# Arief-AK/OpenCL-Development-Real-time-Image-Processing

Hardware: AMD Instinct MI355X
Metric: Mpixels/s (Gaussian 5x5, 4K RGBA) (higher is better)
Workload: dtype u8 in/out, f32 accumulate

## Files before the change

opencl-development-real-time-image-processing_amd/csrc/gauss_exact.hip:

```cpp
#include <type_traits>

#include "common.hpp"
#include "exact_common.hpp"
#include "kernels.hpp"
#include "slide_common.hpp"

namespace mi355 {

namespace {

template <int R, bool CLAMP>
__global__ __launch_bounds__(kSlideWavesPerBlock * 64) void gauss_exact_kernel(
    const uint8_t* __restrict__ in, uint8_t* __restrict__ out, int w, int h, int nstrips, int lanes_out, BandPlan plan,
    ExactTables<2 * R + 1> tab, uint32_t alpha255)
{
    constexpr int K = 2 * R + 1;
    __shared__ float flat[256];
    flat[threadIdx.x] = flat_chain<K>((float)threadIdx.x, tab.w2);
    __syncthreads();
    const int lane = threadIdx.x & 63;
    SlideItem it;
    if (!slide_item(plan, nstrips, h, &it))
        return;
    const bool up = (it.band & 1) != 0;
    const SlideGeom G = slide_geom<4>(it.strip, lanes_out, lane, w, 16u, 16u);
    const BandWalk W = band_walk(up, it.y0, it.nout, R, h);
    const int nin = W.nin, nout = it.nout;

    const size_t row_bytes = (size_t)w * 4;
    const auto fin = uniform_ptr(in + it.frame * row_bytes * h);
    const auto fout = uniform_ptr(out + it.frame * row_bytes * h);
    uint32_t in_off = G.in_off, out_off = G.out_off;

    float wv[R + 1];
#pragma unroll
    for (int d = 0; d <= R; d++)
        wv[d] = tab.w1[R - d];
// ... 85 lines not shown
    constexpr int K = 2 * R + 1;
    const StripPlan sp = make_strip_plan(w);
    BandPlan plan;
    constexpr int kRows = (R == 1) ? 16 : (R == 2 ? 24 : 40);
    constexpr int kWavesPerSimd = (R == 1) ? 5 : (R == 2 ? 3 : 2);
    if (!make_band_plan(h, sp.nstrips, nframes, kWavesPerSimd, kRows, kRows, kRows, 0.0, kRows / 2, &plan))
        return hipErrorInvalidValue;
    double wsum;
    const ExactTables<K> tab = make_exact_tables<K>(coef, &wsum);
    float chain = 0.0f;
    for (int j = 0; j < K * K; j++)
        chain += 255.0f * coef.h_w2d[j];
    chain = chain < 0.0f ? 0.0f : (chain > 255.0f ? 255.0f : chain);
    const uint32_t alpha255 = (uint32_t)chain << 24;
    return dispatch_bool(gauss_upper_clamp(wsum, 0.01), [&](auto CL) {
        return launch_slide(gauss_exact_kernel<R, CL.value>, plan, stream, d_in, d_out, w, h, sp.nstrips, sp.lanes_out,
                            plan, tab, alpha255);
    });
}

}

bool gauss_exact_supported(const uint8_t* d_in, const uint8_t* d_out, int w, int h, const GaussCoef& coef)
{
    (void)h;
    const int k = coef.k;
    if (k != 3 && k != 5 && k != 7)
        return false;
    if (rows_ragged(w, d_in, 16, d_out, 16))
        return false;
    return exact_tables_ok(coef);
}
// ... 10 lines not shown
```

opencl-development-real-time-image-processing_amd/csrc/gauss_slide.hip:

```cpp
#include <cmath>
#include <cstdlib>
#include <type_traits>

#include "common.hpp"
#include "kernels.hpp"
#include "slide_common.hpp"

namespace mi355 {

namespace {

constexpr uint32_t kRowStoreNowhere = 0x80000000u;
__device__ __forceinline__ void gstore_row_nt(global_ptr<uint8_t> rowp, uint32_t row_bytes, uint32_t off, u32x4 v)
{
    const auto rsrc = __builtin_amdgcn_make_buffer_rsrc((void*)rowp, (short)0, (int)row_bytes, 0x00020000);
    __builtin_amdgcn_raw_buffer_store_b128(v, rsrc, (int)off, 0, 2 );
}

constexpr uint32_t kSlideLdsForFiveWaves = 160u * 1024u / 5u - 1024u;
template <typename... KArgs, typename... Args>
hipError_t launch_slide_lds(void (*kernel)(KArgs...), const BandPlan& plan, uint32_t lds_bytes, hipStream_t stream,
                            Args... args)
{
    hipLaunchKernelGGL(kernel, dim3(plan.nblocks_a + plan.nblocks_b), dim3(kSlideWavesPerBlock * 64), lds_bytes, stream,
                       static_cast<KArgs>(args)...);
    return hipGetLastError();
}

template <int K>
struct Weights {
    float w[K];
};

__device__ __forceinline__ float ubyte_f32(uint32_t p, int c)
{
    return (float)((p >> (8 * c)) & 0xFFu);
}

__device__ __forceinline__ void cvt_pack4x4(const float (&h)[4][4] , u32x4& o)
{
    uint32_t o0, o1, o2, o3;
    asm("v_cvt_u32_f32_e32 %0, %4\n\t"
// ... 94 lines not shown
        : "=&v"(o0), "=&v"(o1), "=&v"(o2), "=&v"(o3)
        : "v"(v0), "v"(v1), "v"(v2), "v"(v3), "v"(w0), "v"(w1), "v"(w2), "v"(w3), "v"(w4));
}

struct SlideLane {
    global_ptr<const uint8_t> fin;
    global_ptr<uint8_t> fout;
    size_t row_bytes;
    SlideGeom g;
    int y0, nout, h;
    uint32_t px_off[4];
    int w;
    RaggedEdge edge;
};

template <bool NA0>
__device__ __forceinline__ bool alpha_row_differs(const u32x4& p, uint32_t nA)
{
    uint32_t t;
    if constexpr (NA0)
        t = (p.x & p.y) & (p.z & p.w);
    else
        t = ((p.x ^ nA) & (p.y ^ nA)) & ((p.z ^ nA) & (p.w ^ nA));
    return __builtin_amdgcn_ballot_w64(t < 0xFF000000u) != 0;
}

constexpr int kBandDone = 0;
constexpr int kBandAbortUniform = 1;
constexpr int kBandAbort = 2;
constexpr int kBandAbortUniformFirst = 3;
// ... 12 lines not shown

template <int R, bool CLAMP, int NCH, bool RAGGED, bool UP, int AMODE, bool LOCKSTEP>
__device__ __forceinline__ int gauss_slide_band(const SlideLane& L, const float (&wv)[2 * R + 1], uint32_t alpha_hi,
                                                const uint32_t* __restrict__ alpha_tab, u32x4 (&q3)[2 * R + 1],
                                                bool preloaded)
{
    constexpr int K = 2 * R + 1;
    static_assert((NCH == 4) == (AMODE == 0), "AMODE 1 / 2 belong to the 3-channel pass");
    uint32_t in_off = L.g.in_off, out_off = L.g.out_off;
    [[maybe_unused]] const uint32_t out_voff = L.g.stores ? out_off : kRowStoreNowhere;
    const BandWalk W = band_walk(UP, L.y0, L.nout, R, L.h);
    uint32_t cur_nA = 0u;
    int run = 0;
    int code = kBandDone;
    const ptrdiff_t step_bytes = UP ? -(ptrdiff_t)L.row_bytes : (ptrdiff_t)L.row_bytes;
    const int y_lo = max(L.y0 - R, 0), y_hi = min(L.y0 + L.nout - 1 + R, L.h - 1);
    int y_in = W.y_first;
    auto in_p = L.fin + (size_t)clampi(y_in, y_lo, y_hi) * L.row_bytes;
    auto out_p = L.fout + (size_t)out_row(W, 0) * L.row_bytes;
    auto next_in_row = [&]() {
        const int y_next = y_in + W.y_step;
        in_p += (min(y_in, y_next) >= y_lo && max(y_in, y_next) <= y_hi) ? step_bytes : (ptrdiff_t)0;
        y_in = y_next;
    };
    auto load_row = [&]() -> u32x4 {
        const auto rowp = in_p;
        next_in_row();
        if constexpr (R <= 2)
            lane_offset_here(in_off);
        if constexpr (RAGGED) {
            if (L.w < 4) {
                u32x4 r;
#pragma unroll
                for (int j = 0; j < 4; j++)
                    r[j] = gload<uint32_t>(rowp + L.px_off[j]);
                return r;
            }
            return gload_a4<u32x4>(rowp + in_off);
        } else {
            return gload<u32x4>(rowp + in_off);
        }
    };

    constexpr int PF = (K < 3) ? K : 3;
    u32x4 q_own[K];
    u32x4 (&q)[K] = (AMODE == 0) ? q_own : q3;
    if (AMODE != 2 || !preloaded) {
#pragma unroll
        for (int u = 0; u < PF; u++)
            q[u] = load_row();
    } else {
#pragma unroll
        for (int u = 0; u < PF; u++)
            next_in_row();
    }
    if constexpr (AMODE == 1) {
        if (alpha_row_differs<true>(q[0], 0u)) {
            const uint32_t a_row = ((uint32_t)__builtin_amdgcn_readfirstlane((int)q[0].x) >> 24) & 0xFFu;
            return alpha_row_differs<false>(q[0], (a_row ^ 0xFFu) << 24) ? kBandAbort : kBandAbortUniformFirst;
        }
    }

    constexpr bool kRing = R <= 3;
    static_assert(kRing || !UP, "the accumulator form walks down only");
    float rows[K][4 * NCH] = {};

    auto do_row = [&](auto slot, auto outputs) __attribute__((always_inline)) {
        constexpr int u = decltype(slot)::value;
        constexpr bool OUT = decltype(outputs)::value;
// ... 162 lines not shown
        constexpr int V = decltype(v)::value;
        if constexpr (V < K - 1) {
            if (V < rem) {
                do_row(std::integral_constant<int, (2 * R + V) % K>{}, std::true_type{});
                self(self, std::integral_constant<int, V + 1>{});
            }
        }
    };
    if (code == kBandDone)
        rem_rows(rem_rows, std::integral_constant<int, 0>{});
    return code;
}

template <int R, bool CLAMP, bool RAGGED, int MODE, bool LOCKSTEP>
__global__ __launch_bounds__(kSlideWavesPerBlock * 64, (R == 3 && MODE == 3) ? 3 : 1) void gauss_slide_kernel(
    const uint8_t* __restrict__ in, uint8_t* __restrict__ out, int w, int h, int nstrips, int lanes_out,
    BandPlan plan, Weights<2 * R + 1> wts, uint32_t alpha_hi, const uint32_t* __restrict__ alpha_tab,
    uint32_t* __restrict__ flags)
{
    constexpr int K = 2 * R + 1;
    const int lane = threadIdx.x & 63;
    SlideItem it;
    if (!slide_item(plan, nstrips, h, &it))
        return;
    if constexpr (MODE == 4) {
        if (flags[it.work] == 0)
            return;
    }
    SlideLane L;
    L.g = slide_geom<4>(it.strip, lanes_out, lane, w, 16u, 16u);
    L.y0 = it.y0;
    L.nout = it.nout;
    L.h = h;
    L.w = w;
    L.row_bytes = (size_t)w * 4;
    L.fin = uniform_ptr(in + it.frame * L.row_bytes * h);
    L.fout = uniform_ptr(out + it.frame * L.row_bytes * h);
    L.edge = RaggedEdge{false, false, false, false};
    if constexpr (RAGGED) {
        if (w >= 4)
            L.g.in_off = ragged_edge_setup(L.g.q_lane, L.g.q_load, w, &L.edge);
    }
#pragma unroll
    for (int j = 0; j < 4; j++)
        L.px_off[j] = (uint32_t)clampi(L.g.x_lane + j, 0, w - 1) * 4u;

    float wv[K];
#pragma unroll
    for (int j = 0; j < K; j++) {
        wv[j] = wts.w[j];
        asm volatile("" : "+v"(wv[j]));
    }

    const bool up = (it.band & 1) != 0;
    u32x4 q3[K];
    auto run = [&](auto amode, bool preloaded) -> int {
        constexpr int AMODE = decltype(amode)::value;
        constexpr int NCH = AMODE == 0 ? 4 : 3;
        if constexpr (R <= 3) {
            if (up)
                return gauss_slide_band<R, CLAMP, NCH, RAGGED, true, AMODE, LOCKSTEP>(L, wv, alpha_hi, alpha_tab, q3, preloaded);
        }
        return gauss_slide_band<R, CLAMP, NCH, RAGGED, false, AMODE, LOCKSTEP>(L, wv, alpha_hi, alpha_tab, q3, preloaded);
    };
    auto three_channels = [&]() -> int {
        int code = run(std::integral_constant<int, 1>{}, false);
        if (code == kBandAbortUniform || code == kBandAbortUniformFirst)
            code = run(std::integral_constant<int, 2>{}, code == kBandAbortUniformFirst);
        return code;
    };
    if constexpr (MODE == 0) {
        if (three_channels() != kBandDone)
            run(std::integral_constant<int, 0>{}, false);
    } else if constexpr (MODE == 3) {
        const int code = three_channels();
        if (lane == 0)
            flags[it.work] = code == kBandDone ? 0u : 1u;
    } else {
        run(std::integral_constant<int, 0>{}, false);
    }
}
// ... 26 lines not shown
    const int nstrips = sp.nstrips, lanes_out = sp.lanes_out;
    Weights<K> wts;
    for (int j = 0; j < K; j++)
        wts.w[j] = coef.h_w1d[j];
    double wsum = 0.0;
    for (int j = 0; j < K; j++)
        wsum += (double)coef.h_w1d[j];
    if (!coef.d_alpha_tab)
        return hipErrorInvalidValue;
    const uint32_t alpha_hi = coef.h_alpha_tab[255];
    const uint32_t* alpha_tab = coef.d_alpha_tab;
    const bool lockstep =
        R <= 2 && !ragged && nstrips % kSlideWavesPerBlock == 0 && plan.nwork_b == 0 && plan.nwork_a >= 8192u;
    const uint32_t lds_bytes = (R == 1 && !ragged) ? kSlideLdsForFiveWaves : 0u;
    auto launch = [&](auto kernel) {
        return launch_slide_lds(kernel, plan, lds_bytes, stream, d_in, d_out, w, h, nstrips, lanes_out, plan, wts, alpha_hi,
                                alpha_tab, d_flags);
    };
    return dispatch_bool(gauss_upper_clamp(wsum), [&](auto CL) {
        return dispatch_bool(ragged, [&](auto RG) {
            if constexpr (kSplit) {
                const hipError_t e = launch(gauss_slide_kernel<R, CL.value, RG.value, 3, false>);
                return e != hipSuccess ? e : launch(gauss_slide_kernel<R, CL.value, RG.value, 4, false>);
            } else if constexpr (RG.value) {
                return launch(gauss_slide_kernel<R, CL.value, true, 0, false>);
            } else {
                return dispatch_bool(
                    lockstep, [&](auto LS) { return launch(gauss_slide_kernel<R, CL.value, false, 0, LS.value>); });
            }
        });
    });
}
// ... 32 lines not shown
```

opencl-development-real-time-image-processing_amd/csrc/gauss_wide.hip:

```cpp
#include <cmath>

#include "common.hpp"
#include "kernels.hpp"
#include "slide_common.hpp"

namespace mi355 {

namespace {

template <int K>
struct WWeights {
    float w[K];
};

struct WideLane {
    const uint8_t* fin;
    uint8_t* fout;
    f32x4* vr;
    size_t row_bytes;
    SlideGeom g;
    int y0, nout, nin, h, lane;
};

template <int R, int NCH>
// ... 80 lines not shown
                    for (int c = 0; c < NCH; c++) {
                        r.x = __builtin_amdgcn_cvt_pk_u8_f32(__builtin_floorf(o0[c]), (uint32_t)c, r.x);
                        r.y = __builtin_amdgcn_cvt_pk_u8_f32(__builtin_floorf(o1[c]), (uint32_t)c, r.y);
                    }
                    __builtin_nontemporal_store(
                        r, reinterpret_cast<u32x2*>(L.fout + (size_t)out_row(W, m) * L.row_bytes + L.g.out_off));
                }
            }
        }
    }
    return true;
}

template <int R, int NCH>
__global__ __launch_bounds__(kSlideWavesPerBlock * 64, (NCH == 3 && R <= 6) ? 3 : 2) void gauss_wide_kernel(
    const uint8_t* __restrict__ in, uint8_t* __restrict__ out, int pairs , int h, int nstrips,
    int lanes_out, BandPlan plan, WWeights<2 * R + 1> wts, uint32_t alpha_hi, uint32_t* __restrict__ flags)
{
    constexpr int K = 2 * R + 1;
    constexpr int H = (R + 1) / 2;
    __shared__ f32x4 vrow[kSlideWavesPerBlock][128 + 2 * R + 2];
    SlideItem it;
    if (!slide_item(plan, nstrips, h, &it))
        return;
    if constexpr (NCH == 4) {
        if (flags[it.work] == 0)
            return;
    }
    WideLane L;
    L.vr = vrow[threadIdx.x >> 6];
    L.lane = threadIdx.x & 63;
    L.g = slide_geom<2, H, false>(it.strip, lanes_out, L.lane, 2 * pairs, 8u, 8u);
    L.y0 = it.y0;
    L.nout = it.nout;
    L.nin = it.nout + 2 * R;
    L.h = h;
    L.row_bytes = (size_t)pairs * 8;
    L.fin = in + it.frame * L.row_bytes * h;
// ... 26 lines not shown
hipError_t launch_r(hipStream_t stream, const uint8_t* d_in, uint8_t* d_out, int w, int h, int nframes,
                    const GaussCoef& coef, uint32_t* d_flags)
{
    constexpr int K = 2 * R + 1;
    int pairs, nstrips, lanes_out;
    BandPlan plan;
    if (!d_flags || !wide_plan<R>(w, h, nframes, pairs, nstrips, lanes_out, &plan))
        return hipErrorInvalidValue;
    WWeights<K> wts;
    for (int j = 0; j < K; j++)
        wts.w[j] = coef.h_w1d[j];
    if (!coef.d_alpha_tab)
        return hipErrorInvalidValue;
    const uint32_t alpha_hi = coef.h_alpha_tab[255];
    auto launch = [&](auto kernel) {
        return launch_slide(kernel, plan, stream, d_in, d_out, pairs, h, nstrips, lanes_out, plan, wts, alpha_hi,
                            d_flags);
    };
    const hipError_t e = launch(gauss_wide_kernel<R, 3>);
    return e != hipSuccess ? e : launch(gauss_wide_kernel<R, 4>);
}

}

bool gauss_wide_supported(const uint8_t* d_in, const uint8_t* d_out, int w, int h, int k)
{
    (void)h;
    if (k != 11 && k != 13 && k != 15 && k != 17)
        return false;
    if ((w & 1) != 0)
        return false;
    return aligned_to(d_in, 8) && aligned_to(d_out, 8);
// ... 25 lines not shown
```

opencl-development-real-time-image-processing_amd/csrc/gray.hip:

```cpp
#include <cstdlib>

#include "common.hpp"
#include "kernels.hpp"
#include "slide_common.hpp"

namespace mi355 {

namespace {

constexpr int kGrayThreads = 256;
constexpr int kGrayIlp = 4;

__device__ __forceinline__ uint32_t luma_fast_u32(uint32_t px) { return (uint32_t)luma_px_fast(px); }

__device__ __forceinline__ uint32_t pack4(uint32_t a, uint32_t b, uint32_t c, uint32_t d)
{
    return a | (b << 8) | (c << 16) | (d << 24);
}

template <bool ONE_CH>
__global__ __launch_bounds__(kGrayThreads) void gray_vec_kernel(const u32x4* __restrict__ in,
                                                                void* __restrict__ out,
                                                                size_t nquads)
{
// ... 27 lines not shown
        if constexpr (ONE_CH) {
            reinterpret_cast<uint32_t*>(out)[i] = pack4(g0, g1, g2, g3);
        } else {
            u32x4 o;
            o.x = gray_to_rgba(g0);
            o.y = gray_to_rgba(g1);
            o.z = gray_to_rgba(g2);
            o.w = gray_to_rgba(g3);
            reinterpret_cast<u32x4*>(out)[i] = o;
        }
    }
}

template <bool ONE_CH>
__global__ __launch_bounds__(kSlideWavesPerBlock * 64) void gray_strip_kernel(
    const uint8_t* __restrict__ in, uint8_t* __restrict__ out, int quads, int h, int nstrips, BandPlan plan)
{
    SlideItem it;
    if (!slide_item(plan, nstrips, h, &it))
        return;
    const int lane = threadIdx.x & 63;
    const int q = it.strip * 64 + lane;
    if (q >= quads)
        return;
    const size_t row_in = (size_t)quads * 16, row_out = ONE_CH ? (size_t)quads * 4 : row_in;
    const auto fin = uniform_ptr(in + it.frame * row_in * h);
    const auto fout = uniform_ptr(out + it.frame * row_out * h);
    uint32_t in_off = (uint32_t)q * 16u, out_off = (uint32_t)q * (ONE_CH ? 4u : 16u);
    constexpr int U = 4;
    for (int r0 = 0; r0 < it.nout; r0 += U) {
        u32x4 p[U];
#pragma unroll
        for (int u = 0; u < U; u++) {
            const int y = it.y0 + min(r0 + u, it.nout - 1);
// ... 63 lines not shown
        return (e && atoi(e) > 0) ? (unsigned)atoi(e) : (1u << 20);
    }();
    static const bool kStripForced = tune_env("MI355_TUNE_GRAY_STRIP") != nullptr;
    static const int kStripRows = [] {
        const char* e = tune_env("MI355_TUNE_GRAY_STRIP");
        return e ? atoi(e) : 4;
    }();
    const int strip_quads = w / 4, strip_n = (strip_quads + 63) / 64;
    const bool strip_ok = (w & 3) == 0 && (kStripForced || (strip_quads * 100 >= strip_n * 64 * 93 && npx >= ((size_t)1 << 28)));
    if (nquads && kStripRows > 0 && strip_ok) {
        const int quads = strip_quads, nstrips = strip_n;
        BandPlan plan;
        if (!make_band_plan(h, nstrips, nframes, 8, kStripRows, kStripRows, kStripRows, 0.0, 0, &plan))
            return hipErrorInvalidValue;
        return dispatch_bool(one_channel, [&](auto ONE_CH) {
            return launch_slide(gray_strip_kernel<ONE_CH.value>, plan, stream, d_in, d_out, quads, h, nstrips, plan);
        });
    }
    if (nquads) {
        const unsigned grid = grid_for(nquads, kGrayThreads * kGrayIlp, kCap);
        if (one_channel)
            hipLaunchKernelGGL(gray_vec_kernel<true>, dim3(grid), dim3(kGrayThreads), 0, stream,
                               reinterpret_cast<const u32x4*>(d_in), (void*)d_out, nquads);
        else
            hipLaunchKernelGGL(gray_vec_kernel<false>, dim3(grid), dim3(kGrayThreads), 0, stream,
                               reinterpret_cast<const u32x4*>(d_in), (void*)d_out, nquads);
    }
    const size_t done = nquads * 4;
    if (done < npx) {
        const unsigned grid = grid_for(npx - done, kGrayThreads, kCap);
        if (one_channel)
// ... 11 lines not shown
```

opencl-development-real-time-image-processing_amd/csrc/pipe_slide.hip:

```cpp
#include <cmath>
#include <cstdlib>

#include "common.hpp"
#include "kernels.hpp"
#include "slide_common.hpp"
#include "exact_common.hpp"

namespace mi355 {

namespace {

template <int PX>
struct PixRow {
    u32x4 v[PX / 4];
};

template <int R, int PX, bool CLAMP, bool RAGGED>
__global__ __launch_bounds__(kSlideWavesPerBlock * 64, PX == 8 ? 4 : 1) void pipe_slide_kernel(
    const uint8_t* __restrict__ in, uint8_t* __restrict__ out, int w, int h, int nstrips,
    int lanes_out, BandPlan plan, ExactTables<2 * R + 1> tab)
{
    static_assert(PX == 4 || (PX == 8 && !RAGGED), "8 pixels per lane: aligned rows only");
    constexpr int K = 2 * R + 1;
    __shared__ uint8_t lut[256];
    __shared__ float flat[256];
    lut[threadIdx.x] = (uint8_t)luma_rgb(threadIdx.x, threadIdx.x, threadIdx.x);
    flat[threadIdx.x] = flat_chain<K>((float)threadIdx.x, tab.w2);
    __syncthreads();

    const int lane = threadIdx.x & 63;
    SlideItem it;
    if (!slide_item(plan, nstrips, h, &it))
        return;
    const int y0 = it.y0, nout = it.nout;
    const bool up = (it.band & 1) != 0;

    const SlideGeom G = slide_geom<PX>(it.strip, lanes_out, lane, w, 4u * PX, (uint32_t)PX);
    const int jw = w - G.x_lane;
    const int keep_px = (lane == 0) ? PX - 1 : ((G.q_lane == G.q_end) ? 0 : -1);

    const BandWalk W = band_walk(up, y0, nout, R + 1, h);
    const int nin = W.nin;

    const size_t row_bytes = (size_t)w * 4;
    const auto fin = uniform_ptr(in + it.frame * row_bytes * h);
    const auto fout = uniform_ptr(out + it.frame * (size_t)w * h);
    uint32_t in_off = G.in_off, out_off = G.out_off;
// ... 194 lines not shown
    } else {
        const StripPlan sp = make_strip_plan(w);
        nstrips = sp.nstrips;
        lanes_out = sp.lanes_out;
        constexpr int kRows = (R == 1) ? 16 : (R == 2 ? 24 : 40);
        planned = make_band_plan(h, nstrips, nframes, 8, kRows, kRows, kRows, 0.0, kRows / 2, &plan);
    }
    if (!planned)
        return hipErrorInvalidValue;
    double wsum;
    const ExactTables<K> tab = make_exact_tables<K>(coef, &wsum);
    const bool ragged = PX == 4 && rows_ragged(w, d_in, 16, d_out, 4);
    return dispatch_bool(gauss_upper_clamp(wsum), [&](auto CL) {
        return dispatch_bool(ragged, [&](auto RG) {
            if constexpr (PX == 4 || !RG.value)
                return launch_slide(pipe_slide_kernel<R, PX, CL.value, RG.value>, plan, stream, d_in, d_out, w, h,
                                    nstrips, lanes_out, plan, tab);
            else
                return hipErrorInvalidValue;
        });
    });
}

}

bool pipe_slide_supported(const uint8_t* d_in, const uint8_t* d_out, int w, int h, const GaussCoef& coef, int px)
{
    const int k = coef.k;
    if (k != 3 && k != 5 && k != 7)
        return false;
    if (w < 4 || h < 2 || !exact_tables_ok(coef) || !aligned_to(d_in, 4))
        return false;
// ... 22 lines not shown
```

opencl-development-real-time-image-processing_amd/csrc/slide_common.hpp:

```cpp
#pragma once
#include <cstdint>
#include <cstdlib>

#include "common.hpp"

namespace mi355 {

constexpr int kSlideLanesOutMax = 62;
constexpr int kSlideWavesPerBlock = 4;

struct BandPlan {
    int rows_a, nbands_a, rows_b, nbands_b, y_split;
    uint32_t nwork_a, nwork_b, nblocks_a, nblocks_b;
};

struct StripPlan {
    int quads, nstrips, lanes_out;
};

inline StripPlan make_strip_plan(int w, int lanes_pref = 0)
{
    StripPlan s;
    s.quads = (w + 3) / 4;
    s.nstrips = (s.quads + kSlideLanesOutMax - 1) / kSlideLanesOutMax;
    s.lanes_out = (s.quads + s.nstrips - 1) / s.nstrips;
    if (lanes_pref > 0 && lanes_pref <= kSlideLanesOutMax && s.nstrips > 1) {
        s.lanes_out = lanes_pref;
        s.nstrips = (s.quads + lanes_pref - 1) / lanes_pref;
// ... 47 lines not shown
    p.y_split = h_a;
    if (h_b > 0) {
        p.nbands_b = (h_b + rows_tail - 1) / rows_tail;
        p.rows_b = (h_b + p.nbands_b - 1) / p.nbands_b;
    } else {
        p.nbands_b = 0;
        p.rows_b = 1;
    }
    const size_t na = (size_t)nstrips * p.nbands_a * nframes, nb = (size_t)nstrips * p.nbands_b * nframes;
    if (na + nb > 0x3FFFFFFFull)
        return false;
    p.nwork_a = (uint32_t)na;
    p.nwork_b = (uint32_t)nb;
    p.nblocks_a = (p.nwork_a + kSlideWavesPerBlock - 1) / kSlideWavesPerBlock;
    p.nblocks_b = (p.nwork_b + kSlideWavesPerBlock - 1) / kSlideWavesPerBlock;
    *out = p;
    return true;
}

#ifdef __HIPCC__
template <typename... KArgs, typename... Args>
hipError_t launch_slide(void (*kernel)(KArgs...), const BandPlan& plan, hipStream_t stream, Args... args)
{
    hipLaunchKernelGGL(kernel, dim3(plan.nblocks_a + plan.nblocks_b), dim3(kSlideWavesPerBlock * 64), 0, stream,
                       static_cast<KArgs>(args)...);
    return hipGetLastError();
}

template <typename T>
using global_ptr = __attribute__((address_space(1))) T*;

template <typename T>
__device__ __forceinline__ global_ptr<T> uniform_ptr(T* p)
{
    const uint64_t v = reinterpret_cast<uint64_t>(p);
    const uint32_t lo = __builtin_amdgcn_readfirstlane((uint32_t)v);
    const uint32_t hi = __builtin_amdgcn_readfirstlane((uint32_t)(v >> 32));
    return (global_ptr<T>)(((uint64_t)hi << 32) | lo);
}

__device__ __forceinline__ void lane_offset_here(uint32_t& off)
// ... 41 lines not shown
    const int shift = 4 * q_lane - xs;
    e->sh1 = shift >= 1;
    e->sh2 = shift >= 2;
    e->sh3 = shift >= 3;
    e->sh4 = shift >= 4;
    return (uint32_t)xs * 4u;
}

__device__ __forceinline__ void ragged_shift_clamp(u32x4& p, const RaggedEdge& e)
{
    p.x = e.sh3 ? p.w : (e.sh2 ? p.z : (e.sh1 ? p.y : p.x));
    p.y = e.sh2 ? p.w : (e.sh1 ? p.z : p.y);
    p.z = e.sh1 ? p.w : p.z;
}

struct SlideItem {
    int strip, band, y0, nout;
    uint32_t work;
    size_t frame;
};

__device__ __forceinline__ bool slide_item(const BandPlan& plan, int nstrips, int h, SlideItem* it)
{
    const bool tail = blockIdx.x >= plan.nblocks_a;
    const uint32_t blk = tail ? xcd_remap(blockIdx.x - plan.nblocks_a, plan.nblocks_b)
                              : xcd_remap(blockIdx.x, plan.nblocks_a);
    const uint32_t work =
        __builtin_amdgcn_readfirstlane(blk * kSlideWavesPerBlock + (uint32_t)(threadIdx.x >> 6));
    if (work >= (tail ? plan.nwork_b : plan.nwork_a))
        return false;
    const int nbands = tail ? plan.nbands_b : plan.nbands_a;
    const int band_rows = tail ? plan.rows_b : plan.rows_a;
    it->work = tail ? plan.nwork_a + work : work;
    it->strip = work % nstrips;
    const int band = (work / nstrips) % nbands;
    it->frame = work / ((uint32_t)nstrips * nbands);
    it->band = band;
    it->y0 = (tail ? plan.y_split : 0) + band * band_rows;
    it->nout = min(band_rows, (tail ? h : plan.y_split) - it->y0);
    return true;
}

struct SlideGeom {
    int q_lane, q_load, q_end, x_lane;
    bool left_of_image, right_of_image, edge_strip, stores;
    uint32_t in_off, out_off;
};

template <int PX, int HALO = 1, bool CAP_LOAD = true>
__device__ __forceinline__ SlideGeom slide_geom(int strip, int lanes_out, int lane, int w, uint32_t bytes_in,
                                                uint32_t bytes_out)
{
    static_assert(HALO == 1 || !CAP_LOAD, "the cap is written for one halo lane");
    const int quads = (w + PX - 1) >> (PX == 8 ? 3 : (PX == 4 ? 2 : 1));
    SlideGeom g;
    g.q_lane = strip * lanes_out + lane - HALO;
    g.q_load = clampi(g.q_lane, 0, CAP_LOAD ? min(quads - 1, (strip + 1) * lanes_out) : quads - 1);
    g.q_end = min((strip + 1) * lanes_out, quads);
    g.x_lane = PX * g.q_lane;
    g.left_of_image = g.q_lane < 0;
    g.right_of_image = g.q_lane >= quads;
    g.edge_strip = (strip == 0) || (PX * (strip * lanes_out + 64 - HALO) > w);
    g.stores = (lane >= HALO) && (g.q_lane < g.q_end);
    g.in_off = (uint32_t)g.q_load * bytes_in;
    g.out_off = (uint32_t)(g.stores ? g.q_lane : 0) * bytes_out;
    return g;
}

struct BandWalk {
    int y_first, y_step, halo, nin, h;
};

// ... 68 lines not shown
```

opencl-development-real-time-image-processing_amd/csrc/sobel_slide.hip:

```cpp
#include <cstdlib>

#include "common.hpp"
#include "kernels.hpp"
#include "slide_common.hpp"

namespace mi355 {

namespace {

template <bool RAGGED, bool LOCKSTEP>
__global__ __launch_bounds__(kSlideWavesPerBlock * 64) void sobel_slide_kernel(
    const uint8_t* __restrict__ in, uint8_t* __restrict__ out, int w, int h, int nstrips, int lanes_out,
    BandPlan plan)
{
    constexpr int K = 3;
    const int lane = threadIdx.x & 63;
    SlideItem it;
    __shared__ uint8_t gray_lut[256];
    fill_gray_lut(gray_lut);
    __syncthreads();
    if (!slide_item(plan, nstrips, h, &it))
        return;
    const SlideGeom G = slide_geom<4>(it.strip, lanes_out, lane, w, 16u, 4u);

    const size_t row_bytes = (size_t)w * 4;
    const auto fin = uniform_ptr(in + it.frame * row_bytes * h);
    const auto fout = uniform_ptr(out + it.frame * (size_t)w * h);
    uint32_t in_off = G.in_off, out_off = G.out_off;
    uint32_t px_off[4];
    ragged_px_offsets<kBorderReflect101>(G.x_lane, w, px_off);

    const BandWalk W = band_walk((it.band & 1) != 0, it.y0, it.nout, 1, h);
    const int nin = W.nin, nout = it.nout;
    auto load_row = [&](int i) -> u32x4 {
        const auto rowp = fin + (size_t)in_row<kBorderReflect101>(W, i) * row_bytes;
        lane_offset_here(in_off);
// ... 67 lines not shown


__device__ __forceinline__ uint32_t luma_px_uniform(uint32_t px, const uint8_t* gray_lut)
{
    const uint32_t r = px & 0xFFu, g = (px >> 8) & 0xFFu, b = (px >> 16) & 0xFFu;
    const uint32_t S = 299u * r + 587u * g + 114u * b;
    constexpr uint32_t M = 4294968u;
    uint32_t q = (uint32_t)(((uint64_t)S * M) >> 32);
    const uint32_t low = S * M;
    if (low < 1000000u)
        q = __builtin_amdgcn_readfirstlane(luma_px_ambiguous(px, gray_lut));
    return q;
}

__global__ __launch_bounds__(kSlideWavesPerBlock * 64) void sobel_strip_kernel(
    const uint8_t* __restrict__ in, uint8_t* __restrict__ out, int quads, int h, int nstrips, BandPlan plan)
{
    constexpr int K = 3;
    const int lane = threadIdx.x & 63;
    SlideItem it;
    __shared__ uint8_t gray_lut[256];
    fill_gray_lut(gray_lut);
    __syncthreads();
    if (!slide_item(plan, nstrips, h, &it))
        return;
    const int w = 4 * quads, nout = it.nout;
    const int q = it.strip * 64 + lane;
    const int q_last = min((it.strip + 1) * 64, quads) - 1;
    const bool active = q <= q_last;
    const bool partial = q_last - it.strip * 64 < 63;
    const int x_left = reflect101(4 * it.strip * 64 - 1, w);
    const int x_right = reflect101(4 * (q_last + 1), w);

    const size_t row_bytes = (size_t)w * 4;
    const auto fin = uniform_ptr(in + it.frame * row_bytes * h);
    const auto fout = uniform_ptr(out + it.frame * (size_t)w * h);
    uint32_t in_off = (uint32_t)min(q, q_last) * 16u;
    uint32_t out_off = (uint32_t)min(q, q_last) * 4u;
    const BandWalk W = band_walk((it.band & 1) != 0, it.y0, it.nout, 1, h);
// ... 75 lines not shown

hipError_t launch_sobel_slide(hipStream_t stream, const uint8_t* d_in, uint8_t* d_out, int w, int h, int nframes)
{
    static const int kStripMode = [] {
        const char* e = tune_env("MI355_TUNE_SOBEL_STRIP");
        return e ? atoi(e) : 1;
    }();
    const bool kStripOff = kStripMode == 0;
    const bool big = (size_t)w * h * nframes >= ((size_t)1 << 28) || kStripMode == 2;
    const bool ragged = rows_ragged(w, d_in, 16, d_out, 4);
    if (!kStripOff && big && !ragged) {
        const int quads = w / 4, nstrips = (quads + 63) / 64;
        BandPlan plan;
        if (!make_band_plan(h, nstrips, nframes, 8, 16, 16, 16, 0.0, 8, &plan))
            return hipErrorInvalidValue;
        return launch_slide(sobel_strip_kernel, plan, stream, d_in, d_out, quads, h, nstrips, plan);
    }
    const StripPlan sp = make_strip_plan(w, big ? 48 : 0);
    BandPlan plan;
    if (!make_band_plan(h, sp.nstrips, nframes, 8, 16, 16, 16, 0.0, 8, &plan))
        return hipErrorInvalidValue;
    const bool lockstep = !ragged && !big && (size_t)w * h * nframes >= 80000000ull;
    auto launch = [&](auto kernel) {
        return launch_slide(kernel, plan, stream, d_in, d_out, w, h, sp.nstrips, sp.lanes_out, plan);
    };
    return ragged ? launch(sobel_slide_kernel<true, false>)
                  : (lockstep ? launch(sobel_slide_kernel<false, true>) : launch(sobel_slide_kernel<false, false>));
}

}
```

Baseline: 783,400.

## Precompute slide work-decode divisors on host and issue first rows before setup

Kernel arguments are reshaped into a flat packed header. Work-item decoding now uses host-precomputed multiply-shift reciprocals in place of runtime integer divides and modulos, and the XCD remap constants are precomputed as well. In the gauss slide kernel, the first prefetch rows are issued through a new RowCursor before the remaining geometry setup, so load latency overlaps the prologue math. This adds a larger argument list and a preloaded path whose correctness depends on the AMODE handling.

New measurement: 786,100, median of 4. Within noise of the previous version (+0.3%).

```diff
diff --git a/opencl-development-real-time-image-processing_amd/csrc/gauss_exact.hip b/opencl-development-real-time-image-processing_amd/csrc/gauss_exact.hip
--- a/opencl-development-real-time-image-processing_amd/csrc/gauss_exact.hip
+++ b/opencl-development-real-time-image-processing_amd/csrc/gauss_exact.hip
@@ -11,16 +11,19 @@
 
 template <int R, bool CLAMP>
 __global__ __launch_bounds__(kSlideWavesPerBlock * 64) void gauss_exact_kernel(
-    const uint8_t* __restrict__ in, uint8_t* __restrict__ out, int w, int h, int nstrips, int lanes_out, BandPlan plan,
+    const uint8_t* __restrict__ in, MI355_SLIDE_HEAD_PARAMS, uint8_t* __restrict__ out,
     ExactTables<2 * R + 1> tab, uint32_t alpha255)
 {
     constexpr int K = 2 * R + 1;
+    const SlideHead hd = MI355_SLIDE_HEAD;
+    const SlidePhase tail = MI355_SLIDE_TAIL;
+    const int w = (int)hd.w, h = (int)hd.h, lanes_out = slide_lanes_out(hd);
     __shared__ float flat[256];
     flat[threadIdx.x] = flat_chain<K>((float)threadIdx.x, tab.w2);
     __syncthreads();
     const int lane = threadIdx.x & 63;
     SlideItem it;
-    if (!slide_item(plan, nstrips, h, &it))
+    if (!slide_item(hd, tail, &it))
         return;
     const bool up = (it.band & 1) != 0;
     const SlideGeom G = slide_geom<4>(it.strip, lanes_out, lane, w, 16u, 16u);
@@ -136,8 +139,8 @@
     chain = chain < 0.0f ? 0.0f : (chain > 255.0f ? 255.0f : chain);
     const uint32_t alpha255 = (uint32_t)chain << 24;
     return dispatch_bool(gauss_upper_clamp(wsum, 0.01), [&](auto CL) {
-        return launch_slide(gauss_exact_kernel<R, CL.value>, plan, stream, d_in, d_out, w, h, sp.nstrips, sp.lanes_out,
-                            plan, tab, alpha255);
+        return launch_slide(gauss_exact_kernel<R, CL.value>, plan, 0u, stream, d_in, w, h, sp.lanes_out, d_out, tab,
+                            alpha255);
     });
 }
 
diff --git a/opencl-development-real-time-image-processing_amd/csrc/gauss_slide.hip b/opencl-development-real-time-image-processing_amd/csrc/gauss_slide.hip
--- a/opencl-development-real-time-image-processing_amd/csrc/gauss_slide.hip
+++ b/opencl-development-real-time-image-processing_amd/csrc/gauss_slide.hip
@@ -18,14 +18,6 @@
 }
 
 constexpr uint32_t kSlideLdsForFiveWaves = 160u * 1024u / 5u - 1024u;
-template <typename... KArgs, typename... Args>
-hipError_t launch_slide_lds(void (*kernel)(KArgs...), const BandPlan& plan, uint32_t lds_bytes, hipStream_t stream,
-                            Args... args)
-{
-    hipLaunchKernelGGL(kernel, dim3(plan.nblocks_a + plan.nblocks_b), dim3(kSlideWavesPerBlock * 64), lds_bytes, stream,
-                       static_cast<KArgs>(args)...);
-    return hipGetLastError();
-}
 
 template <int K>
 struct Weights {
@@ -150,6 +142,32 @@
     RaggedEdge edge;
 };
 
+struct RowCursor {
+    global_ptr<const uint8_t> p;
+    int y, y_lo, y_hi, y_step;
+    ptrdiff_t step_bytes;
+    __device__ __forceinline__ void next()
+    {
+        const int y_next = y + y_step;
+        p += (min(y, y_next) >= y_lo && max(y, y_next) <= y_hi) ? step_bytes : (ptrdiff_t)0;
+        y = y_next;
+    }
+};
+
+template <int R>
+__device__ __forceinline__ RowCursor band_cursor(global_ptr<const uint8_t> fin, size_t row_bytes, int y0, int nout, int h,
+                                                 bool up)
+{
+    RowCursor c;
+    c.y_lo = max(y0 - R, 0);
+    c.y_hi = min(y0 + nout - 1 + R, h - 1);
+    c.y = up ? y0 + nout - 1 + R : y0 - R;
+    c.y_step = up ? -1 : 1;
+    c.step_bytes = up ? -(ptrdiff_t)row_bytes : (ptrdiff_t)row_bytes;
+    c.p = fin + (size_t)clampi(c.y, c.y_lo, c.y_hi) * row_bytes;
+    return c;
+}
+
 template <bool NA0>
 __device__ __forceinline__ bool alpha_row_differs(const u32x4& p, uint32_t nA)
 {
@@ -192,18 +210,11 @@
     int run = 0;
     int code = kBandDone;
     const ptrdiff_t step_bytes = UP ? -(ptrdiff_t)L.row_bytes : (ptrdiff_t)L.row_bytes;
-    const int y_lo = max(L.y0 - R, 0), y_hi = min(L.y0 + L.nout - 1 + R, L.h - 1);
-    int y_in = W.y_first;
-    auto in_p = L.fin + (size_t)clampi(y_in, y_lo, y_hi) * L.row_bytes;
+    RowCursor C = band_cursor<R>(L.fin, L.row_bytes, L.y0, L.nout, L.h, UP);
     auto out_p = L.fout + (size_t)out_row(W, 0) * L.row_bytes;
-    auto next_in_row = [&]() {
-        const int y_next = y_in + W.y_step;
-        in_p += (min(y_in, y_next) >= y_lo && max(y_in, y_next) <= y_hi) ? step_bytes : (ptrdiff_t)0;
-        y_in = y_next;
-    };
     auto load_row = [&]() -> u32x4 {
-        const auto rowp = in_p;
-        next_in_row();
+        const auto rowp = C.p;
+        C.next();
         if constexpr (R <= 2)
             lane_offset_here(in_off);
         if constexpr (RAGGED) {
@@ -223,14 +234,14 @@
     constexpr int PF = (K < 3) ? K : 3;
     u32x4 q_own[K];
     u32x4 (&q)[K] = (AMODE == 0) ? q_own : q3;
-    if (AMODE != 2 || !preloaded) {
+    if (AMODE == 0 || !preloaded) {
 #pragma unroll
         for (int u = 0; u < PF; u++)
             q[u] = load_row();
     } else {
 #pragma unroll
         for (int u = 0; u < PF; u++)
-            next_in_row();
+            C.next();
     }
     if constexpr (AMODE == 1) {
         if (alpha_row_differs<true>(q[0], 0u)) {
@@ -423,33 +434,55 @@
 
 template <int R, bool CLAMP, bool RAGGED, int MODE, bool LOCKSTEP>
 __global__ __launch_bounds__(kSlideWavesPerBlock * 64, (R == 3 && MODE == 3) ? 3 : 1) void gauss_slide_kernel(
-    const uint8_t* __restrict__ in, uint8_t* __restrict__ out, int w, int h, int nstrips, int lanes_out,
-    BandPlan plan, Weights<2 * R + 1> wts, uint32_t alpha_hi, const uint32_t* __restrict__ alpha_tab,
-    uint32_t* __restrict__ flags)
+    const uint8_t* __restrict__ in, MI355_SLIDE_HEAD_PARAMS, uint8_t* __restrict__ out,
+    Weights<2 * R + 1> wts, uint32_t alpha_hi, const uint32_t* __restrict__ alpha_tab, uint32_t* __restrict__ flags)
 {
     constexpr int K = 2 * R + 1;
+    constexpr int PF = (K < 3) ? K : 3;
+    const SlideHead hd = MI355_SLIDE_HEAD;
+    const SlidePhase tail = MI355_SLIDE_TAIL;
+    const int w = (int)hd.w, h = (int)hd.h, lanes_out = slide_lanes_out(hd);
     const int lane = threadIdx.x & 63;
     SlideItem it;
-    if (!slide_item(plan, nstrips, h, &it))
+    if (!slide_item(hd, tail, &it))
         return;
     if constexpr (MODE == 4) {
         if (flags[it.work] == 0)
             return;
     }
+    const bool up = R <= 3 && (it.band & 1) != 0;
     SlideLane L;
-    L.g = slide_geom<4>(it.strip, lanes_out, lane, w, 16u, 16u);
     L.y0 = it.y0;
     L.nout = it.nout;
     L.h = h;
     L.w = w;
     L.row_bytes = (size_t)w * 4;
     L.fin = uniform_ptr(in + it.frame * L.row_bytes * h);
-    L.fout = uniform_ptr(out + it.frame * L.row_bytes * h);
     L.edge = RaggedEdge{false, false, false, false};
+    uint32_t in_off = slide_geom_load<4>(it.strip, lanes_out, lane, w) * 16u;
     if constexpr (RAGGED) {
         if (w >= 4)
-            L.g.in_off = ragged_edge_setup(L.g.q_lane, L.g.q_load, w, &L.edge);
-    }
+            in_off = ragged_edge_setup(it.strip * lanes_out + lane - 1, (int)(in_off / 16u), w, &L.edge);
+    }
+    u32x4 q3[K];
+    const bool rows_issued = MODE != 4 && R != 3 && !LOCKSTEP && (!RAGGED || w >= 4);
+    if (rows_issued) {
+        RowCursor C = band_cursor<R>(L.fin, L.row_bytes, L.y0, L.nout, h, up);
+        if constexpr (R <= 2)
+            lane_offset_here(in_off);
+#pragma unroll
+        for (int u = 0; u < PF; u++) {
+            if constexpr (RAGGED)
+                q3[u] = gload_a4<u32x4>(C.p + in_off);
+            else
+                q3[u] = gload<u32x4>(C.p + in_off);
+            C.next();
+        }
+        __builtin_amdgcn_sched_barrier(0);
+    }
+    L.g = slide_geom<4>(it.strip, lanes_out, lane, w, 16u, 16u);
+    L.g.in_off = in_off;
+    L.fout = uniform_ptr(out + it.frame * L.row_bytes * h);
 #pragma unroll
     for (int j = 0; j < 4; j++)
         L.px_off[j] = (uint32_t)clampi(L.g.x_lane + j, 0, w - 1) * 4u;
@@ -461,8 +494,6 @@
         asm volatile("" : "+v"(wv[j]));
     }
 
-    const bool up = (it.band & 1) != 0;
-    u32x4 q3[K];
     auto run = [&](auto amode, bool preloaded) -> int {
         constexpr int AMODE = decltype(amode)::value;
         constexpr int NCH = AMODE == 0 ? 4 : 3;
@@ -473,7 +504,7 @@
         return gauss_slide_band<R, CLAMP, NCH, RAGGED, false, AMODE, LOCKSTEP>(L, wv, alpha_hi, alpha_tab, q3, preloaded);
     };
     auto three_channels = [&]() -> int {
-        int code = run(std::integral_constant<int, 1>{}, false);
+        int code = run(std::integral_constant<int, 1>{}, rows_issued);
         if (code == kBandAbortUniform || code == kBandAbortUniformFirst)
             code = run(std::integral_constant<int, 2>{}, code == kBandAbortUniformFirst);
         return code;
@@ -530,8 +561,8 @@
         R <= 2 && !ragged && nstrips % kSlideWavesPerBlock == 0 && plan.nwork_b == 0 && plan.nwork_a >= 8192u;
     const uint32_t lds_bytes = (R == 1 && !ragged) ? kSlideLdsForFiveWaves : 0u;
     auto launch = [&](auto kernel) {
-        return launch_slide_lds(kernel, plan, lds_bytes, stream, d_in, d_out, w, h, nstrips, lanes_out, plan, wts, alpha_hi,
-                                alpha_tab, d_flags);
+        return launch_slide(kernel, plan, lds_bytes, stream, d_in, w, h, lanes_out, d_out, wts, alpha_hi, alpha_tab,
+                            d_flags);
     };
     return dispatch_bool(gauss_upper_clamp(wsum), [&](auto CL) {
         return dispatch_bool(ragged, [&](auto RG) {
diff --git a/opencl-development-real-time-image-processing_amd/csrc/gauss_wide.hip b/opencl-development-real-time-image-processing_amd/csrc/gauss_wide.hip
--- a/opencl-development-real-time-image-processing_amd/csrc/gauss_wide.hip
+++ b/opencl-development-real-time-image-processing_amd/csrc/gauss_wide.hip
@@ -118,14 +118,17 @@
 
 template <int R, int NCH>
 __global__ __launch_bounds__(kSlideWavesPerBlock * 64, (NCH == 3 && R <= 6) ? 3 : 2) void gauss_wide_kernel(
-    const uint8_t* __restrict__ in, uint8_t* __restrict__ out, int pairs , int h, int nstrips,
-    int lanes_out, BandPlan plan, WWeights<2 * R + 1> wts, uint32_t alpha_hi, uint32_t* __restrict__ flags)
-{
+    const uint8_t* __restrict__ in, MI355_SLIDE_HEAD_PARAMS ,
+    uint8_t* __restrict__ out, WWeights<2 * R + 1> wts, uint32_t alpha_hi, uint32_t* __restrict__ flags)
+{
+    const SlideHead hd = MI355_SLIDE_HEAD;
+    const SlidePhase tail = MI355_SLIDE_TAIL;
+    const int pairs = (int)hd.w, h = (int)hd.h, lanes_out = slide_lanes_out(hd);
     constexpr int K = 2 * R + 1;
     constexpr int H = (R + 1) / 2;
     __shared__ f32x4 vrow[kSlideWavesPerBlock][128 + 2 * R + 2];
     SlideItem it;
-    if (!slide_item(plan, nstrips, h, &it))
+    if (!slide_item(hd, tail, &it))
         return;
     if constexpr (NCH == 4) {
         if (flags[it.work] == 0)
@@ -182,8 +185,7 @@
         return hipErrorInvalidValue;
     const uint32_t alpha_hi = coef.h_alpha_tab[255];
     auto launch = [&](auto kernel) {
-        return launch_slide(kernel, plan, stream, d_in, d_out, pairs, h, nstrips, lanes_out, plan, wts, alpha_hi,
-                            d_flags);
+        return launch_slide(kernel, plan, 0u, stream, d_in, pairs, h, lanes_out, d_out, wts, alpha_hi, d_flags);
     };
     const hipError_t e = launch(gauss_wide_kernel<R, 3>);
     return e != hipSuccess ? e : launch(gauss_wide_kernel<R, 4>);
diff --git a/opencl-development-real-time-image-processing_amd/csrc/gray.hip b/opencl-development-real-time-image-processing_amd/csrc/gray.hip
--- a/opencl-development-real-time-image-processing_amd/csrc/gray.hip
+++ b/opencl-development-real-time-image-processing_amd/csrc/gray.hip
@@ -65,10 +65,13 @@
 
 template <bool ONE_CH>
 __global__ __launch_bounds__(kSlideWavesPerBlock * 64) void gray_strip_kernel(
-    const uint8_t* __restrict__ in, uint8_t* __restrict__ out, int quads, int h, int nstrips, BandPlan plan)
+    const uint8_t* __restrict__ in, MI355_SLIDE_HEAD_PARAMS , uint8_t* __restrict__ out)
 {
+    const SlideHead hd = MI355_SLIDE_HEAD;
+    const SlidePhase tail = MI355_SLIDE_TAIL;
+    const int quads = (int)hd.w, h = (int)hd.h;
     SlideItem it;
-    if (!slide_item(plan, nstrips, h, &it))
+    if (!slide_item(hd, tail, &it))
         return;
     const int lane = threadIdx.x & 63;
     const int q = it.strip * 64 + lane;
@@ -162,7 +165,7 @@
         if (!make_band_plan(h, nstrips, nframes, 8, kStripRows, kStripRows, kStripRows, 0.0, 0, &plan))
             return hipErrorInvalidValue;
         return dispatch_bool(one_channel, [&](auto ONE_CH) {
-            return launch_slide(gray_strip_kernel<ONE_CH.value>, plan, stream, d_in, d_out, quads, h, nstrips, plan);
+            return launch_slide(gray_strip_kernel<ONE_CH.value>, plan, 0u, stream, d_in, quads, h, 0, d_out);
         });
     }
     if (nquads) {
diff --git a/opencl-development-real-time-image-processing_amd/csrc/pipe_slide.hip b/opencl-development-real-time-image-processing_amd/csrc/pipe_slide.hip
--- a/opencl-development-real-time-image-processing_amd/csrc/pipe_slide.hip
+++ b/opencl-development-real-time-image-processing_amd/csrc/pipe_slide.hip
@@ -17,9 +17,12 @@
 
 template <int R, int PX, bool CLAMP, bool RAGGED>
 __global__ __launch_bounds__(kSlideWavesPerBlock * 64, PX == 8 ? 4 : 1) void pipe_slide_kernel(
-    const uint8_t* __restrict__ in, uint8_t* __restrict__ out, int w, int h, int nstrips,
-    int lanes_out, BandPlan plan, ExactTables<2 * R + 1> tab)
-{
+    const uint8_t* __restrict__ in, MI355_SLIDE_HEAD_PARAMS, uint8_t* __restrict__ out,
+    ExactTables<2 * R + 1> tab)
+{
+    const SlideHead hd = MI355_SLIDE_HEAD;
+    const SlidePhase tail = MI355_SLIDE_TAIL;
+    const int w = (int)hd.w, h = (int)hd.h, lanes_out = slide_lanes_out(hd);
     static_assert(PX == 4 || (PX == 8 && !RAGGED), "8 pixels per lane: aligned rows only");
     constexpr int K = 2 * R + 1;
     __shared__ uint8_t lut[256];
@@ -30,7 +33,7 @@
 
     const int lane = threadIdx.x & 63;
     SlideItem it;
-    if (!slide_item(plan, nstrips, h, &it))
+    if (!slide_item(hd, tail, &it))
         return;
     const int y0 = it.y0, nout = it.nout;
     const bool up = (it.band & 1) != 0;
@@ -255,8 +258,8 @@
     return dispatch_bool(gauss_upper_clamp(wsum), [&](auto CL) {
         return dispatch_bool(ragged, [&](auto RG) {
             if constexpr (PX == 4 || !RG.value)
-                return launch_slide(pipe_slide_kernel<R, PX, CL.value, RG.value>, plan, stream, d_in, d_out, w, h,
-                                    nstrips, lanes_out, plan, tab);
+                return launch_slide(pipe_slide_kernel<R, PX, CL.value, RG.value>, plan, 0u, stream, d_in, w, h,
+                                    lanes_out, d_out, tab);
             else
                 return hipErrorInvalidValue;
         });
diff --git a/opencl-development-real-time-image-processing_amd/csrc/slide_common.hpp b/opencl-development-real-time-image-processing_amd/csrc/slide_common.hpp
--- a/opencl-development-real-time-image-processing_amd/csrc/slide_common.hpp
+++ b/opencl-development-real-time-image-processing_amd/csrc/slide_common.hpp
@@ -9,9 +9,40 @@
 constexpr int kSlideLanesOutMax = 62;
 constexpr int kSlideWavesPerBlock = 4;
 
+#ifdef __HIPCC__
+#define MI355_HD __host__ __device__
+#else
+#define MI355_HD
+#endif
+#ifdef __HIP_DEVICE_COMPILE__
+#define MI355_OPAQUE_U32(x) asm volatile("" : "+s"(x))
+#else
+#define MI355_OPAQUE_U32(x) asm volatile("" : "+r"(x))
+#endif
+struct DivU30 {
+    uint32_t mul, shift;
+};
+
+MI355_HD inline DivU30 make_div_u30(uint32_t d)
+{
+    d = d ? d : 1u;
+    uint32_t l = 0;
+    while (((uint64_t)1 << l) < d)
+        l++;
+    return DivU30{(uint32_t)((((uint64_t)1 << (30 + l)) + d - 1) / d), l};
+}
+
+MI355_HD inline uint32_t div_u30(uint32_t n, uint32_t mul, uint32_t shift)
+{
+    return (uint32_t)(((uint64_t)(n << 2) * mul) >> 32) >> shift;
+}
+
 struct BandPlan {
     int rows_a, nbands_a, rows_b, nbands_b, y_split;
     uint32_t nwork_a, nwork_b, nblocks_a, nblocks_b;
+    int nstrips;
+    DivU30 div_strips, div_bands_a, div_bands_b, div_item_a, div_item_b;
+    uint32_t xcd_q_a, xcd_r_a, xcd_q_b, xcd_r_b;
 };
 
 struct StripPlan {
@@ -89,17 +120,115 @@
     p.nwork_b = (uint32_t)nb;
     p.nblocks_a = (p.nwork_a + kSlideWavesPerBlock - 1) / kSlideWavesPerBlock;
     p.nblocks_b = (p.nwork_b + kSlideWavesPerBlock - 1) / kSlideWavesPerBlock;
+    p.nstrips = nstrips;
+    p.div_strips = make_div_u30((uint32_t)nstrips);
+    p.div_bands_a = make_div_u30((uint32_t)p.nbands_a);
+    p.div_bands_b = make_div_u30((uint32_t)p.nbands_b);
+    p.div_item_a = make_div_u30((uint32_t)nstrips * p.nbands_a);
+    p.div_item_b = make_div_u30((uint32_t)nstrips * p.nbands_b);
+    p.xcd_q_a = p.nblocks_a >> 3;
+    p.xcd_r_a = p.nblocks_a & 7u;
+    p.xcd_q_b = p.nblocks_b >> 3;
+    p.xcd_r_b = p.nblocks_b & 7u;
     *out = p;
     return true;
 }
 
+struct SlidePhase {
+    uint32_t nwork, nbands, rows, y_base, y_end;
+    uint32_t xcd_q, mul_item;
+    uint32_t bits;
+};
+
+struct SlideHead {
+    uint32_t w, h;
+    uint32_t geo;
+    uint32_t nstrips, mul_strips, nblocks_a;
+    uint32_t nwork_a, nbands_a, rows_a, y_split, xcd_q_a, mul_item_a;
+};
+#define MI355_SLIDE_HEAD_PARAMS                                                                                        \
+    uint32_t sh_w, uint32_t sh_h, uint32_t sh_geo, uint32_t sh_nstrips, uint32_t sh_mul_strips, uint32_t sh_nblocks_a, \
+        uint32_t sh_nwork_a, uint32_t sh_nbands_a, uint32_t sh_rows_a, uint32_t sh_y_split, uint32_t sh_xcd_q_a,       \
+        uint32_t sh_mul_item_a, uint32_t st_nwork, uint32_t st_nbands, uint32_t st_rows, uint32_t st_y_base,           \
+        uint32_t st_y_end, uint32_t st_xcd_q, uint32_t st_mul_item, uint32_t st_bits
+#define MI355_SLIDE_HEAD                                                                                         \
+    SlideHead { sh_w, sh_h, sh_geo, sh_nstrips, sh_mul_strips, sh_nblocks_a, sh_nwork_a, sh_nbands_a, sh_rows_a, \
+                sh_y_split, sh_xcd_q_a, sh_mul_item_a }
+#define MI355_SLIDE_TAIL \
+    SlidePhase { st_nwork, st_nbands, st_rows, st_y_base, st_y_end, st_xcd_q, st_mul_item, st_bits }
+
+MI355_HD inline int slide_lanes_out(const SlideHead& hd) { return (int)(hd.geo & 0xFFu); }
+
+inline SlideHead make_slide_head(const BandPlan& p, int w, int h, int lanes_out)
+{
+    const uint32_t bits_a = p.div_item_a.shift | p.xcd_r_a << 8;
+    return SlideHead{(uint32_t)w, (uint32_t)h, (uint32_t)lanes_out | p.div_strips.shift << 8 | bits_a << 16,
+                     (uint32_t)p.nstrips, p.div_strips.mul, p.nblocks_a, p.nwork_a, (uint32_t)p.nbands_a,
+                     (uint32_t)p.rows_a, (uint32_t)p.y_split, p.xcd_q_a, p.div_item_a.mul};
+}
+
+inline SlidePhase make_slide_tail(const BandPlan& p, int h)
+{
+    return SlidePhase{p.nwork_b, (uint32_t)p.nbands_b, (uint32_t)p.rows_b, (uint32_t)p.y_split, (uint32_t)h,
+                      p.xcd_q_b, p.div_item_b.mul, p.div_item_b.shift | p.xcd_r_b << 8};
+}
+
+MI355_HD inline uint32_t slide_block_work(const SlideHead& hd, const SlidePhase& tail, uint32_t bid, SlidePhase* ph,
+                                          uint32_t* first)
+{
+    *ph = SlidePhase{hd.nwork_a, hd.nbands_a, hd.rows_a, 0u, hd.y_split, hd.xcd_q_a, hd.mul_item_a, hd.geo >> 16};
+    *first = 0u;
+    if (bid >= hd.nblocks_a) {
+        uint32_t f[8] = {tail.nwork, tail.nbands, tail.rows, tail.y_base, tail.y_end, tail.xcd_q, tail.mul_item, tail.bits};
+        for (int j = 0; j < 8; j++)
+            MI355_OPAQUE_U32(f[j]);
+        *ph = SlidePhase{f[0], f[1], f[2], f[3], f[4], f[5], f[6], f[7]};
+        *first = hd.nwork_a;
+        bid -= hd.nblocks_a;
+    }
+    const uint32_t xcd = bid & 7u, r = (ph->bits >> 8) & 7u;
+    return ((bid >> 3) + xcd * ph->xcd_q + (xcd < r ? xcd : r)) * (uint32_t)kSlideWavesPerBlock;
+}
+
+struct SlideItem {
+    int strip, band, y0, nout;
+    uint32_t work;
+    size_t frame;
+};
+
+MI355_HD inline void slide_decode_work(const SlideHead& hd, const SlidePhase& ph, uint32_t first, uint32_t work,
+                                       SlideItem* it)
+{
+    const uint32_t t = div_u30(work, hd.mul_strips, (hd.geo >> 8) & 31u);
+    const uint32_t frame = div_u30(work, ph.mul_item, ph.bits & 31u);
+    const uint32_t band = t - frame * ph.nbands;
+    const uint32_t y0 = ph.y_base + band * ph.rows;
+    it->work = first + work;
+    it->strip = (int)(work - t * hd.nstrips);
+    it->band = (int)band;
+    it->frame = frame;
+    it->y0 = (int)y0;
+    it->nout = (int)(ph.rows < ph.y_end - y0 ? ph.rows : ph.y_end - y0);
+}
+
 #ifdef __HIPCC__
 template <typename... KArgs, typename... Args>
-hipError_t launch_slide(void (*kernel)(KArgs...), const BandPlan& plan, hipStream_t stream, Args... args)
-{
-    hipLaunchKernelGGL(kernel, dim3(plan.nblocks_a + plan.nblocks_b), dim3(kSlideWavesPerBlock * 64), 0, stream,
-                       static_cast<KArgs>(args)...);
+hipError_t launch_slide_args(void (*kernel)(KArgs...), dim3 grid, uint32_t lds_bytes, hipStream_t stream, Args... args)
+{
+    hipLaunchKernelGGL(kernel, grid, dim3(kSlideWavesPerBlock * 64), lds_bytes, stream, static_cast<KArgs>(args)...);
     return hipGetLastError();
+}
+
+template <typename... KArgs, typename... Rest>
+hipError_t launch_slide(void (*kernel)(KArgs...), const BandPlan& plan, uint32_t lds_bytes, hipStream_t stream,
+                        const uint8_t* d_in, int w, int h, int lanes_out, Rest... rest)
+{
+    const SlideHead hd = make_slide_head(plan, w, h, lanes_out);
+    const SlidePhase t = make_slide_tail(plan, h);
+    return launch_slide_args(kernel, dim3(plan.nblocks_a + plan.nblocks_b), lds_bytes, stream, d_in, hd.w, hd.h, hd.geo,
+                             hd.nstrips, hd.mul_strips, hd.nblocks_a, hd.nwork_a, hd.nbands_a, hd.rows_a, hd.y_split,
+                             hd.xcd_q_a, hd.mul_item_a, t.nwork, t.nbands, t.rows, t.y_base, t.y_end, t.xcd_q, t.mul_item,
+                             t.bits, rest...);
 }
 
 template <typename T>
@@ -171,30 +300,16 @@
     p.z = e.sh1 ? p.w : p.z;
 }
 
-struct SlideItem {
-    int strip, band, y0, nout;
-    uint32_t work;
-    size_t frame;
-};
-
-__device__ __forceinline__ bool slide_item(const BandPlan& plan, int nstrips, int h, SlideItem* it)
-{
-    const bool tail = blockIdx.x >= plan.nblocks_a;
-    const uint32_t blk = tail ? xcd_remap(blockIdx.x - plan.nblocks_a, plan.nblocks_b)
-                              : xcd_remap(blockIdx.x, plan.nblocks_a);
-    const uint32_t work =
-        __builtin_amdgcn_readfirstlane(blk * kSlideWavesPerBlock + (uint32_t)(threadIdx.x >> 6));
-    if (work >= (tail ? plan.nwork_b : plan.nwork_a))
+__device__ __forceinline__ bool slide_item(const SlideHead& hd, const SlidePhase& tail, SlideItem* it)
+{
+    static_assert(kXcdRun == 0, "slide_block_work restates the contiguous remap");
+    SlidePhase ph;
+    uint32_t first;
+    const uint32_t work0 = slide_block_work(hd, tail, blockIdx.x, &ph, &first);
+    const uint32_t work = __builtin_amdgcn_readfirstlane(work0 + (uint32_t)(threadIdx.x >> 6));
+    if (work >= ph.nwork)
         return false;
-    const int nbands = tail ? plan.nbands_b : plan.nbands_a;
-    const int band_rows = tail ? plan.rows_b : plan.rows_a;
-    it->work = tail ? plan.nwork_a + work : work;
-    it->strip = work % nstrips;
-    const int band = (work / nstrips) % nbands;
-    it->frame = work / ((uint32_t)nstrips * nbands);
-    it->band = band;
-    it->y0 = (tail ? plan.y_split : 0) + band * band_rows;
-    it->nout = min(band_rows, (tail ? h : plan.y_split) - it->y0);
+    slide_decode_work(hd, ph, first, work, it);
     return true;
 }
 
@@ -205,14 +320,21 @@
 };
 
 template <int PX, int HALO = 1, bool CAP_LOAD = true>
+__device__ __forceinline__ int slide_geom_load(int strip, int lanes_out, int lane, int w)
+{
+    static_assert(HALO == 1 || !CAP_LOAD, "the cap is written for one halo lane");
+    const int quads = (w + PX - 1) >> (PX == 8 ? 3 : (PX == 4 ? 2 : 1));
+    return clampi(strip * lanes_out + lane - HALO, 0, CAP_LOAD ? min(quads - 1, (strip + 1) * lanes_out) : quads - 1);
+}
+
+template <int PX, int HALO = 1, bool CAP_LOAD = true>
 __device__ __forceinline__ SlideGeom slide_geom(int strip, int lanes_out, int lane, int w, uint32_t bytes_in,
                                                 uint32_t bytes_out)
 {
-    static_assert(HALO == 1 || !CAP_LOAD, "the cap is written for one halo lane");
     const int quads = (w + PX - 1) >> (PX == 8 ? 3 : (PX == 4 ? 2 : 1));
     SlideGeom g;
     g.q_lane = strip * lanes_out + lane - HALO;
-    g.q_load = clampi(g.q_lane, 0, CAP_LOAD ? min(quads - 1, (strip + 1) * lanes_out) : quads - 1);
+    g.q_load = slide_geom_load<PX, HALO, CAP_LOAD>(strip, lanes_out, lane, w);
     g.q_end = min((strip + 1) * lanes_out, quads);
     g.x_lane = PX * g.q_lane;
     g.left_of_image = g.q_lane < 0;
diff --git a/opencl-development-real-time-image-processing_amd/csrc/sobel_slide.hip b/opencl-development-real-time-image-processing_amd/csrc/sobel_slide.hip
--- a/opencl-development-real-time-image-processing_amd/csrc/sobel_slide.hip
+++ b/opencl-development-real-time-image-processing_amd/csrc/sobel_slide.hip
@@ -10,16 +10,18 @@
 
 template <bool RAGGED, bool LOCKSTEP>
 __global__ __launch_bounds__(kSlideWavesPerBlock * 64) void sobel_slide_kernel(
-    const uint8_t* __restrict__ in, uint8_t* __restrict__ out, int w, int h, int nstrips, int lanes_out,
-    BandPlan plan)
+    const uint8_t* __restrict__ in, MI355_SLIDE_HEAD_PARAMS, uint8_t* __restrict__ out)
 {
     constexpr int K = 3;
+    const SlideHead hd = MI355_SLIDE_HEAD;
+    const SlidePhase tail = MI355_SLIDE_TAIL;
+    const int w = (int)hd.w, h = (int)hd.h, lanes_out = slide_lanes_out(hd);
     const int lane = threadIdx.x & 63;
     SlideItem it;
     __shared__ uint8_t gray_lut[256];
     fill_gray_lut(gray_lut);
     __syncthreads();
-    if (!slide_item(plan, nstrips, h, &it))
+    if (!slide_item(hd, tail, &it))
         return;
     const SlideGeom G = slide_geom<4>(it.strip, lanes_out, lane, w, 16u, 4u);
 
@@ -117,15 +119,18 @@
 }
 
 __global__ __launch_bounds__(kSlideWavesPerBlock * 64) void sobel_strip_kernel(
-    const uint8_t* __restrict__ in, uint8_t* __restrict__ out, int quads, int h, int nstrips, BandPlan plan)
+    const uint8_t* __restrict__ in, MI355_SLIDE_HEAD_PARAMS , uint8_t* __restrict__ out)
 {
     constexpr int K = 3;
+    const SlideHead hd = MI355_SLIDE_HEAD;
+    const SlidePhase tail = MI355_SLIDE_TAIL;
+    const int quads = (int)hd.w, h = (int)hd.h;
     const int lane = threadIdx.x & 63;
     SlideItem it;
     __shared__ uint8_t gray_lut[256];
     fill_gray_lut(gray_lut);
     __syncthreads();
-    if (!slide_item(plan, nstrips, h, &it))
+    if (!slide_item(hd, tail, &it))
         return;
     const int w = 4 * quads, nout = it.nout;
     const int q = it.strip * 64 + lane;
@@ -231,7 +236,7 @@
         BandPlan plan;
         if (!make_band_plan(h, nstrips, nframes, 8, 16, 16, 16, 0.0, 8, &plan))
             return hipErrorInvalidValue;
-        return launch_slide(sobel_strip_kernel, plan, stream, d_in, d_out, quads, h, nstrips, plan);
+        return launch_slide(sobel_strip_kernel, plan, 0u, stream, d_in, quads, h, 0, d_out);
     }
     const StripPlan sp = make_strip_plan(w, big ? 48 : 0);
     BandPlan plan;
@@ -239,7 +244,7 @@
         return hipErrorInvalidValue;
     const bool lockstep = !ragged && !big && (size_t)w * h * nframes >= 80000000ull;
     auto launch = [&](auto kernel) {
-        return launch_slide(kernel, plan, stream, d_in, d_out, w, h, sp.nstrips, sp.lanes_out, plan);
+        return launch_slide(kernel, plan, 0u, stream, d_in, w, h, sp.lanes_out, d_out);
     };
     return ragged ? launch(sobel_slide_kernel<true, false>)
                   : (lockstep ? launch(sobel_slide_kernel<false, true>) : launch(sobel_slide_kernel<false, false>));
```
